# RainbowZL0/swin-unet-image-fusion

Measured on AMD Instinct MI355X. Metric: fused image-pairs/sec at 256x256, win=8, higher is better.
Workload: dtype bf16; 1 GPU; B=16/GPU 256x256 IR/visible pairs, win=8, 5-level Swin-UNet fusion forward (BASELINE configs[1]); global_batch=16, precision_mode=fast, residual_stream=fp32, hip_graph=True, steps_in_flight=3, kernel_schedule=throughput, collective=none, weights=random-init (numpy PCG64 recipe, seed 0)

## Files before the change

swin_unet_image_fusion_amd/csrc/kernels_attnproj.hip:

```cpp
#include "kernels_attnproj.h"

#include <cstdlib>

#include "win_frag.h"

namespace swf {
namespace {

using namespace wf;

constexpr int kC = 384, kD = 48, kHeads = 8, kNS = 3, kVRS = 72, kLDO = kC + 8;
constexpr size_t kVtBytes = size_t(kHeads) * kD * kVRS * 2, kBiasBytes = 2 * 2 * 16 * 64 * 4;
constexpr size_t kOBytes = size_t(2) * 64 * kLDO * 2;
constexpr size_t kXchBytes = size_t(8) * 16 * 64 * 4;
static_assert(kVtBytes + kBiasBytes <= kOBytes, "the O image covers the attention-phase images");
constexpr size_t kLds = kOBytes + kXchBytes;

struct ApDev {
    const f16* q[2]; const f16* k[2]; const f16* v[2];
    const bf16* wp_hi[2]; const bf16* wp_lo[2];
    const float* pbias[2]; const float* table[2];
    const float* res[2]; float* out[2];
    int B, H, W, shift;
};

#ifdef AP_PROBE
__device__ unsigned long long ap_probe[16];
#define AP_STAMP(i) do { if (blockIdx.x == AP_PROBE && blockIdx.y == 0 && blockIdx.z == 0 && threadIdx.x == 0) ap_probe[i] = wall_clock64(); } while (0)
#else
#define AP_STAMP(i) do { } while (0)
#endif

template <int WS>
__global__ __launch_bounds__(512) void attn_proj_kernel(ApDev a) {
    static_assert(WS == 7 || WS == 8, "window side");
    constexpr int C = kC, D = kD, VRS = kVRS, LDO = kLDO, TW = 2 * WS - 1;
    extern __shared__ __attribute__((aligned(16))) char smem[];
    f16* vt = reinterpret_cast<f16*>(smem);
    float* btile = reinterpret_cast<float*>(smem + kVtBytes);
    bf16* o_hi = reinterpret_cast<bf16*>(smem);
    bf16* o_lo = o_hi + 64 * LDO;

    const int tid = threadIdx.x, lane = tid & 63, wave = __builtin_amdgcn_readfirstlane(tid >> 6);
    const int r = lane & 31, hf = lane >> 5;
    const int H = a.H, W = a.W, nwx = W / WS, nwy = H / WS, npi = nwx * nwy;
    const int win = blockIdx.x, ns = blockIdx.y, st = blockIdx.z;
    const int b = win / npi, wrem = win - b * npi, wy = wrem / nwx, wx = wrem - wy * nwx;
    const int sh = a.shift ? WS / 2 : 0;
    auto padding = [](int t) { return WS != 8 && ((t >> 3) >= WS || (t & 7) >= WS); };
    auto tok_index = [&](int t) {
        const int ty = WS == 8 ? (t >> 3) : min(t >> 3, WS - 1), tx = WS == 8 ? (t & 7) : min(t & 7, WS - 1);
        int oy = wy * WS + ty + sh, ox = wx * WS + tx + sh;
        oy = oy >= H ? oy - H : oy;
        ox = ox >= W ? ox - W : ox;
        return (size_t)((b * H + oy) * W + ox);
    };

    AP_STAMP(0);
    const int head = wave;
    const f16* qg = a.q[st] + head * D + 8 * hf;
    const f16* kg = a.k[st] + head * D + 8 * hf;
    const size_t t0 = tok_index(r) * C, t1 = tok_index(32 + r) * C;
    u32x4 kf[2][3], qf[2][3], vrow[6];
#pragma unroll
    for (int ks = 0; ks < 3; ++ks) {
        kf[0][ks] = *reinterpret_cast<const u32x4*>(kg + t0 + 16 * ks);
        kf[1][ks] = *reinterpret_cast<const u32x4*>(kg + t1 + 16 * ks);
        qf[0][ks] = *reinterpret_cast<const u32x4*>(qg + t0 + 16 * ks);
        qf[1][ks] = *reinterpret_cast<const u32x4*>(qg + t1 + 16 * ks);
    }
    {
        const f16* vg = a.v[st] + tok_index(lane) * C + head * D;
#pragma unroll
        for (int j = 0; j < 6; ++j) vrow[j] = *reinterpret_cast<const u32x4*>(vg + 8 * j);
    }
    {
        const bool last_row = a.shift && wy == nwy - 1, last_col = a.shift && wx == nwx - 1;
        const float* tab = a.table[st];
#pragma unroll
// ... 43 lines not shown
#pragma unroll
        for (int i = 3; i < 16; i += 2) mx = max3f(mx, acc[0][i], acc[0][i + 1 < 16 ? i + 1 : i]);
#pragma unroll
        for (int i = 2; i < 16; i += 2) mx = max3f(mx, acc[1][i], acc[1][i + 1]);
        mx = max_halves(mx);
        float l = 0.f;
#pragma unroll
        for (int kt = 0; kt < 2; ++kt)
#pragma unroll
            for (int i = 0; i < 16; ++i) {
                acc[kt][i] = __builtin_amdgcn_exp2f(acc[kt][i] - mx);
                l += acc[kt][i];
            }
        l = sum_halves(l);
        o[qb][0] = zero16;
        o[qb][1] = zero16;
#pragma unroll
        for (int kt = 0; kt < 2; ++kt)
#pragma unroll
            for (int s2 = 0; s2 < 2; ++s2) {
                float p[8];
#pragma unroll
                for (int e = 0; e < 8; ++e) p[e] = acc[kt][8 * s2 + e];
                const u32x4 pf = pack8_f16(p);
                const u32x4 va0 = *reinterpret_cast<const u32x4*>(vth + r * VRS + kt * 32 + s2 * 16);
                const u32x4 va1 = *reinterpret_cast<const u32x4*>(vth + c1 * VRS + kt * 32 + s2 * 16);
                o[qb][0] = mfma_f16(va0, pf, o[qb][0]);
                o[qb][1] = mfma_f16(va1, pf, o[qb][1]);
            }
        inv[qb] = 1.0f / l;
    }

    AP_STAMP(4);
    const int ct = wave & 3, kh = wave >> 2, col0 = ns * (C / kNS) + 32 * ct;
    constexpr int KSH = C / 32;
    u32x4 wfh[KSH], wfl[KSH];
    {
        const size_t blk0 = (size_t)(col0 / 32) * (C / 16) + KSH * kh;
        const bf16* wh = a.wp_hi[st] + blk0 * 512 + lane * 8;
        const bf16* wl = a.wp_lo[st] + blk0 * 512 + lane * 8;
#pragma unroll
        for (int ks = 0; ks < KSH; ++ks) {
            wfh[ks] = *reinterpret_cast<const u32x4*>(wh + 512 * ks);
            wfl[ks] = *reinterpret_cast<const u32x4*>(wl + 512 * ks);
        }
    }
    const int t = 32 * kh + r;
    const size_t orow = tok_index(t) * C + col0 + 4 * hf;
    f32x4 rv[4], bv[4];
#pragma unroll
    for (int g = 0; g < 4; ++g) {
        rv[g] = *reinterpret_cast<const f32x4*>(a.res[st] + orow + 8 * g);
        bv[g] = a.pbias[st] ? *reinterpret_cast<const f32x4*>(a.pbias[st] + col0 + 8 * g + 4 * hf) : f32x4{0.f, 0.f, 0.f, 0.f};
    }
    __syncthreads();
#pragma unroll
    for (int qb = 0; qb < 2; ++qb)
#pragma unroll
        for (int mt = 0; mt < 2; ++mt)
#pragma unroll
            for (int g = 0; g < 4; ++g) {
                const int c = mt * 32 + 8 * g + 4 * hf;
                if (c < D) {
                    bf16x4 h4, l4;
#pragma unroll
                    for (int j = 0; j < 4; ++j) {
                        const float v = o[qb][mt][4 * g + j] * inv[qb];
                        h4[j] = (bf16)v;
                        l4[j] = (bf16)(v - (float)h4[j]);
                    }
                    *reinterpret_cast<bf16x4*>(o_hi + (32 * qb + r) * LDO + head * D + c) = h4;
                    *reinterpret_cast<bf16x4*>(o_lo + (32 * qb + r) * LDO + head * D + c) = l4;
                }
            }
    __syncthreads();
    AP_STAMP(5);

    f32x16 acc[2] = {zero16, zero16};
    {
        const bf16* oh = o_hi + r * LDO + (C / 2) * kh + 8 * hf;
        const bf16* ol = o_lo + r * LDO + (C / 2) * kh + 8 * hf;
#pragma unroll
        for (int ks = 0; ks < KSH; ++ks) {
            const u32x4 bh0 = *reinterpret_cast<const u32x4*>(oh + 16 * ks), bl0 = *reinterpret_cast<const u32x4*>(ol + 16 * ks);
            const u32x4 bh1 = *reinterpret_cast<const u32x4*>(oh + 32 * LDO + 16 * ks), bl1 = *reinterpret_cast<const u32x4*>(ol + 32 * LDO + 16 * ks);
            acc[0] = mma3(wfh[ks], wfl[ks], bh0, bl0, acc[0]);
            acc[1] = mma3(wfh[ks], wfl[ks], bh1, bl1, acc[1]);
        }
    }
    float* xch = reinterpret_cast<float*>(smem + kOBytes);
#pragma unroll
    for (int i = 0; i < 16; ++i) xch[(wave * 16 + i) * 64 + lane] = kh ? acc[0][i] : acc[1][i];
    __syncthreads();
    AP_STAMP(6);
    f32x16 mine = kh ? acc[1] : acc[0];
#pragma unroll
    for (int i = 0; i < 16; ++i) mine[i] += xch[((wave ^ 4) * 16 + i) * 64 + lane];
    if (padding(t)) return;
    float* out = a.out[st] + orow;
#pragma unroll
    for (int g = 0; g < 4; ++g) {
        f32x4 v = {mine[4 * g], mine[4 * g + 1], mine[4 * g + 2], mine[4 * g + 3]};
        v += bv[g];
        v += rv[g];
        *reinterpret_cast<f32x4*>(out + 8 * g) = v;
    }
    AP_STAMP(7);
}

}

bool attnproj_supported(const swf_block_desc& d) {
    static const bool off = debug_env("SWF_NO_ATTNPROJ") != nullptr;
    return !off && d.precision == SWF_PREC_FAST && d.attn.channels == kC && d.attn.heads == kHeads && d.attn.head_dim == kD &&
           d.attn.win_h == d.attn.win_w && (d.attn.win_h == 8 || d.attn.win_h == 7);
}

int launch_attnproj(const swf_block_desc& d, const AttnProjArgs& a, int nstream, hipStream_t stream) {
    const int ws = d.attn.win_h;
    if (!attnproj_supported(d) || a.H % ws || a.W % ws) return fail(SWF_ERR_UNSUPPORTED, "attnproj: shape not covered");
    if ((int64_t)a.B * a.H * a.W > INT32_MAX / kC) return fail(SWF_ERR_UNSUPPORTED, "attnproj: token count");
    ApDev dv{};
    for (int s = 0; s < nstream; ++s) {
        if (!a.q[s] || !a.k[s] || !a.v[s] || !a.wp_hi[s] || !a.wp_lo[s] || !a.table[s] || !a.res[s] || !a.out[s])
            return fail(SWF_ERR_NULL, "attnproj: NULL operand (stream %d)", s);
        dv.q[s] = reinterpret_cast<const f16*>(a.q[s]); dv.k[s] = reinterpret_cast<const f16*>(a.k[s]); dv.v[s] = reinterpret_cast<const f16*>(a.v[s]);
        dv.wp_hi[s] = reinterpret_cast<const bf16*>(a.wp_hi[s]); dv.wp_lo[s] = reinterpret_cast<const bf16*>(a.wp_lo[s]);
        dv.pbias[s] = a.pbias[s]; dv.table[s] = a.table[s]; dv.res[s] = a.res[s]; dv.out[s] = a.out[s];
    }
    dv.B = a.B; dv.H = a.H; dv.W = a.W; dv.shift = a.shift;
    const int nwin = a.B * (a.H / ws) * (a.W / ws);
    if (ws == 8) {
        SWF_TRY(raise_lds_limit<&attn_proj_kernel<8>>((int)kLds, "attn_proj"));
        hipLaunchKernelGGL((attn_proj_kernel<8>), dim3(nwin, kNS, nstream), dim3(512), kLds, stream, dv);
    } else {
        SWF_TRY(raise_lds_limit<&attn_proj_kernel<7>>((int)kLds, "attn_proj"));
        hipLaunchKernelGGL((attn_proj_kernel<7>), dim3(nwin, kNS, nstream), dim3(512), kLds, stream, dv);
    }
    return check_launch("attn_proj");
}

}
```

swin_unet_image_fusion_amd/csrc/kernels_deeppatch.h:

```cpp
#pragma once
#include "kernels_patch.h"

namespace swf {

bool deep_patch_supported(int decoder, int Cin, int Cout, int mh, int mw);
size_t deep_patch_packed_bytes(int decoder, int Cin, int Cout, int mh, int mw);
int pack_deep_patch(int decoder, int Cin, int Cout, int mh, int mw, const float* weight, void* dst, hipStream_t stream);
bool deep_patch_raw(int decoder, int Cin, int Cout, int mh, int mw);
struct DeepPatchExtra {
    const float* ln_gamma[2]; const float* ln_beta[2]; unsigned short* ln_hi[2]; unsigned short* ln_lo[2];
    const void* warm[2]; size_t warm_bytes;
};
int launch_deep_patch(const PatchFusedDesc& d, const void* const* packed, int nstream, hipStream_t stream, float* const* raw_out = nullptr,
                      const DeepPatchExtra* extra = nullptr);

int launch_deep_patch_finish(const PatchFusedDesc& d, float* const* raw, int nstream, hipStream_t stream, const DeepPatchExtra* extra = nullptr);

struct DeepQkvArgs {
    const unsigned short* xn_hi[2]; const unsigned short* xn_lo[2];
    const unsigned short* w_hi[2]; const unsigned short* w_lo[2];
    const float* bias[2][3];
    unsigned short* out[2][3];
    float qscale; int cross, M;
    int C;
};
bool deep_qkv_supported(const swf_block_desc& d);
int launch_deep_qkv(const DeepQkvArgs& q, int nstream, hipStream_t stream);

struct DeepProjArgs {
    const unsigned short* o_hi[2]; const unsigned short* o_lo[2];
    const unsigned short* w_hi[2]; const unsigned short* w_lo[2];
    const float* bias[2]; const float* res[2]; float* out[2];
    int M, C;
};
bool deep_proj_supported(const swf_block_desc& d);
int launch_deep_proj(const DeepProjArgs& q, int nstream, hipStream_t stream);

}
```

swin_unet_image_fusion_amd/csrc/kernels_deeppatch.hip:

```cpp
#include "kernels_deeppatch.h"

#include <cstdlib>

#include "kernels_qkvattn.h"
#include "win_frag.h"

namespace swf {
namespace {

using namespace wf;

struct DpArgs {
    const float* in[2]; float* out[2]; const float* skip[2];
    const bf16* w_hi[2]; const bf16* w_lo[2];
    const float* bias[2]; const float* gamma[2]; const float* beta[2];
    int B, H, W, Hm, Wm, Ho, Wo, M;
    const bf16* xh[2]; const bf16* xl[2]; const float* qb[2][3]; f16* qo[2][3]; float qscale; int cross;
    const float* ln_g[2]; const float* ln_b[2]; bf16* ln_hi[2]; bf16* ln_lo[2];
    const char* warm[2]; int warm_bytes;
};

#ifdef DP_PROBE
__device__ unsigned long long dp_probe[16];
#define DP_STAMP(i) do { if (blockIdx.x == DP_PROBE && blockIdx.y == 0 && threadIdx.x == 0) dp_probe[i] = wall_clock64(); } while (0)
// ... 516 lines not shown
    const int C = d.attn.channels;
    return !off && d.precision == SWF_PREC_FAST && d.attn.heads * d.attn.head_dim == C && (C == 384 || C == 192);
}

int launch_deep_proj(const DeepProjArgs& q, int nstream, hipStream_t stream) {
    if (q.M <= 0 || q.M > INT32_MAX / 2048) return fail(SWF_ERR_UNSUPPORTED, "deep_proj: token count");
    if (q.C != 192 && q.C != 384) return fail(SWF_ERR_UNSUPPORTED, "deep_proj: C=%d", q.C);
    DpArgs a{};
    for (int s = 0; s < nstream; ++s) {
        if (!q.o_hi[s] || !q.o_lo[s] || !q.w_hi[s] || !q.w_lo[s] || !q.out[s]) return fail(SWF_ERR_NULL, "deep_proj: NULL operand (stream %d)", s);
        a.xh[s] = reinterpret_cast<const bf16*>(q.o_hi[s]); a.xl[s] = reinterpret_cast<const bf16*>(q.o_lo[s]);
        a.w_hi[s] = reinterpret_cast<const bf16*>(q.w_hi[s]); a.w_lo[s] = reinterpret_cast<const bf16*>(q.w_lo[s]);
        a.bias[s] = q.bias[s]; a.skip[s] = q.res[s]; a.out[s] = q.out[s];
    }
    a.M = q.M;
    return q.C == 192 ? launch_t<192, 192, 2, 4, 3, 192>(a, nstream, stream) : launch_t<384, 192, 2, 4, 3, 384>(a, nstream, stream);
}

int launch_deep_qkv(const DeepQkvArgs& q, int nstream, hipStream_t stream) {
    if (q.M <= 0 || q.M > INT32_MAX / 2048) return fail(SWF_ERR_UNSUPPORTED, "deep_qkv: token count");
    DpArgs a{};
    for (int s = 0; s < nstream; ++s) {
        if (!q.xn_hi[s] || !q.xn_lo[s] || !q.w_hi[s] || !q.w_lo[s]) return fail(SWF_ERR_NULL, "deep_qkv: NULL operand (stream %d)", s);
        a.xh[s] = reinterpret_cast<const bf16*>(q.xn_hi[s]); a.xl[s] = reinterpret_cast<const bf16*>(q.xn_lo[s]);
        a.w_hi[s] = reinterpret_cast<const bf16*>(q.w_hi[s]); a.w_lo[s] = reinterpret_cast<const bf16*>(q.w_lo[s]);
        for (int i = 0; i < 3; ++i) {
            if (!q.out[s][i]) return fail(SWF_ERR_NULL, "deep_qkv: NULL output (stream %d)", s);
            a.qb[s][i] = q.bias[s][i]; a.qo[s][i] = reinterpret_cast<f16*>(q.out[s][i]);
        }
    }
    a.M = q.M; a.qscale = q.qscale; a.cross = q.cross && nstream == 2;
    if (q.C == 192) return launch_t<192, 192, 2, 4, 2, 576>(a, nstream, stream);
    if (q.C != 384) return fail(SWF_ERR_UNSUPPORTED, "deep_qkv: C=%d", q.C);
    return launch_t<384, 192, 2, 4, 2, 1152>(a, nstream, stream);
}

bool deep_patch_supported(int decoder, int Cin, int Cout, int mh, int mw) { return shape_index(decoder, Cin, Cout, mh, mw) >= 0; }
bool deep_patch_raw(int decoder, int Cin, int Cout, int mh, int mw) {
    const int i = shape_index(decoder, Cin, Cout, mh, mw);
    return i >= 0 && kShapes[i].raw;
}

size_t deep_patch_packed_bytes(int decoder, int Cin, int Cout, int mh, int mw) {
    const int i = shape_index(decoder, Cin, Cout, mh, mw);
    return i < 0 ? 0 : align_up((size_t)kShapes[i].K * kShapes[i].N * 4, 256);
}

int pack_deep_patch(int decoder, int Cin, int Cout, int mh, int mw, const float* weight, void* dst, hipStream_t stream) {
    const int i = shape_index(decoder, Cin, Cout, mh, mw);
    if (i < 0) return fail(SWF_ERR_UNSUPPORTED, "pack_deep_patch: shape not covered");
    const int K = kShapes[i].K, N = kShapes[i].N;
    bf16* hi = static_cast<bf16*>(dst);
    hipLaunchKernelGGL(dp_pack_kernel, dim3(256), dim3(256), 0, stream, weight, hi, hi + (size_t)N * K, N, K);
    return check_launch("pack_deep_patch");
}

int launch_deep_patch(const PatchFusedDesc& d, const void* const* packed, int nstream, hipStream_t stream, float* const* raw_out,
                      const DeepPatchExtra* extra) {
    const int i = shape_index(d.decoder, d.Cin, d.Cout, d.mh, d.mw);
    if (i < 0) return fail(SWF_ERR_UNSUPPORTED, "deep_patch: shape not covered");
    if (d.M <= 0 || d.M > INT32_MAX / 1024 || (int64_t)d.B * d.H * d.W * d.Cin > INT32_MAX) return fail(SWF_ERR_UNSUPPORTED, "deep_patch: map too large");
    const int K = kShapes[i].K, N = kShapes[i].N;
    DpArgs a{};
    for (int s = 0; s < nstream; ++s) {
        if (!packed || !packed[s] || !d.in[s] || !d.out[s] || !d.gamma[s] || !d.beta[s]) return fail(SWF_ERR_NULL, "deep_patch: NULL operand (stream %d)", s);
        if (kShapes[i].raw && (!raw_out || !raw_out[s])) return fail(SWF_ERR_NULL, "deep_patch: this shape needs the conv output buffer (stream %d)", s);
// ... 25 lines not shown
```

swin_unet_image_fusion_amd/csrc/kernels_patchrr.hip:

```cpp
#include "kernels_patchrr.h"

#include <algorithm>

#include "win_frag.h"

namespace swf {
namespace {

using namespace wf;

struct PrrArgs {
    const float* in[2]; float* out[2]; const float* skip[2]; const char* packed[2];
    int B, H, W, Cin;
    int mh, mw, Hm, Wm;
    int Ho, Wo;
    int K, N, Cout, M;
};

template <int KS, int NT>
struct PRR {
    static constexpr int NFRAG = NT * KS * 2;
    static constexpr int NV = NT * 16;
    static constexpr size_t p_vec = size_t(NFRAG) * 1024;
    static constexpr size_t p_total = p_vec + size_t(3) * 2 * NV * 4;
};

template <int KS, int NT, int DEC, int CIN1, int TPW>
__global__ __launch_bounds__(256) void patch_rr_kernel(PrrArgs a) {
    using P = PRR<KS, NT>;
    constexpr int NV = P::NV;
    __shared__ float lvec[3 * 2 * NV];
    const int s = blockIdx.y, tid = threadIdx.x, lane = tid & 63, wave = tid >> 6;
    const int r = lane & 31, hf = lane >> 5;
    fill_vectors<3 * NV / 4, 256>(lvec, a.packed[s] + P::p_vec, a.packed[s] + P::p_vec + (3 * NV / 4) * 16, tid);
    const __amdgpu_buffer_rsrc_t wrs = __builtin_amdgcn_make_buffer_rsrc(const_cast<char*>(a.packed[s]), 0, (int)P::p_total, 0x00020000);
    const unsigned loff = (unsigned)lane * 16u;
    auto WA = [&](int nt, int ks, int hl) {
        return __builtin_bit_cast(u32x4, __builtin_amdgcn_raw_buffer_load_b128(wrs, loff, ((nt * KS + ks) * 2 + hl) * 1024, 0));
    };
    __syncthreads();
    const float* vbias = lvec + hf * NV;
    const float* vgam = lvec + 2 * NV + hf * NV;
    const float* vbet = lvec + 4 * NV + hf * NV;
    const float* in = a.in[s];
    const int K = a.K, N = a.N, Cin = a.Cin;
    const float invN = 1.0f / (float)N;
    const f32x16 zero16 = {0.f, 0.f, 0.f, 0.f, 0.f, 0.f, 0.f, 0.f, 0.f, 0.f, 0.f, 0.f, 0.f, 0.f, 0.f, 0.f};

    const int ngroup = (a.M + 32 * TPW - 1) / (32 * TPW);
    for (int grp = blockIdx.x * 4 + wave; grp < ngroup; grp += gridDim.x * 4) {
        int tok[TPW], base[TPW][4];
        bool live[TPW];
#pragma unroll
        for (int u = 0; u < TPW; ++u) {
            const int t = (grp * TPW + u) * 32 + r;
            live[u] = t < a.M;
            const int tc = live[u] ? t : a.M - 1;
            tok[u] = tc;
            if constexpr (DEC) {
                const int mx = tc % a.Wm, t2 = tc / a.Wm, my = t2 % a.Hm, b = t2 / a.Hm;
                base[u][0] = ((b * a.H + my) * a.W + mx) * Cin;
                base[u][1] = base[u][2] = base[u][3] = 0;
            } else {
// ... 54 lines not shown
        auto dec_offsets = [&](int u) {
            const int t = tok[u];
            const int mx = t % a.Wm, t2 = t / a.Wm, my = t2 % a.Hm, b = t2 / a.Hm;
            int pq = 0, c = 4 * hf;
            while (c >= a.Cout) { c -= a.Cout; ++pq; }
#pragma unroll
            for (int nt = 0; nt < NT; ++nt)
#pragma unroll
                for (int g = 0; g < 4; ++g) {
                    const int yy = my * 2 + (pq >> 1), xx = mx * 2 + (pq & 1);
                    const bool ok = live[u] && 32 * nt + 8 * g + 4 * hf < N && yy < a.Ho && xx < a.Wo;
                    oidx[u][nt][g] = ok ? ((b * a.Ho + yy) * a.Wo + xx) * a.Cout + c : -1;
                    c += 8;
                    while (c >= a.Cout) { c -= a.Cout; ++pq; }
                }
        };
        auto load_skips = [&](int u) {
#pragma unroll
            for (int nt = 0; nt < NT; ++nt)
#pragma unroll
                for (int g = 0; g < 4; ++g)
                    skv[u][nt][g] = (a.skip[s] && oidx[u][nt][g] >= 0) ? *reinterpret_cast<const float4*>(a.skip[s] + oidx[u][nt][g])
                                                                       : make_float4(0.f, 0.f, 0.f, 0.f);
        };
        if constexpr (DEC_VEC) {
            if (a.Cout > 1) {
#pragma unroll
                for (int u = 0; u < TPW; ++u) {
                    dec_offsets(u);
                    if constexpr (SKIP_EARLY) load_skips(u);
                }
            }
        }
        u32x4 wr[2][NT][2];
        SWF_WF_FENCE();
#pragma unroll
        for (int nt = 0; nt < NT; ++nt) { wr[0][nt][0] = WA(nt, 0, 0); wr[0][nt][1] = WA(nt, 0, 1); }
#pragma unroll
        for (int ks = 0; ks < KS; ++ks) {
            if (ks + 1 < KS) {
#pragma unroll
                for (int nt = 0; nt < NT; ++nt) { wr[(ks + 1) & 1][nt][0] = WA(nt, ks + 1, 0); wr[(ks + 1) & 1][nt][1] = WA(nt, ks + 1, 1); }
            }
            SWF_WF_FENCE();
            u32x4 bh[TPW], bl[TPW];
#pragma unroll
            for (int u = 0; u < TPW; ++u) split8(xin[u][ks], bh[u], bl[u]);
#pragma unroll
            for (int nt = 0; nt < NT; ++nt)
#pragma unroll
                for (int u = 0; u < TPW; ++u) acc[u][nt] = mma3(wr[ks & 1][nt][0], wr[ks & 1][nt][1], bh[u], bl[u], acc[u][nt]);
        }
#pragma unroll
        for (int u = 0; u < TPW; ++u) {
            float sum = 0.f;
#pragma unroll
            for (int nt = 0; nt < NT; ++nt)
#pragma unroll
                for (int i = 0; i < 16; ++i) {
                    acc[u][nt][i] += vbias[nt * 16 + i];
                    sum += acc[u][nt][i];
                }
            const float mean = sum_halves(sum) * invN;
            float q = 0.f;
#pragma unroll
            for (int nt = 0; nt < NT; ++nt)
#pragma unroll
                for (int i = 0; i < 16; ++i) {
                    const float d = acc[u][nt][i] - mean;
                    q += (32 * nt + rho(i, hf) < N) ? d * d : 0.f;
                }
            const float rstd = __builtin_amdgcn_rsqf(sum_halves(q) * invN + 1e-5f);
            const int t = tok[u];
            if constexpr (DEC_VEC) {
                if (a.Cout > 1) {
                    if constexpr (!SKIP_EARLY) load_skips(u);
                }
            }
#pragma unroll
            for (int nt = 0; nt < NT; ++nt)
#pragma unroll
                for (int g = 0; g < 4; ++g) {
                    const int n0 = 32 * nt + 8 * g + 4 * hf;
                    if (n0 < N) {
// ... 39 lines not shown
    const int gtid = blockIdx.x * blockDim.x + threadIdx.x, gsz = gridDim.x * blockDim.x;
    for (int idx = gtid; idx < P::NFRAG * 512; idx += gsz) {
        const int f = idx >> 9, lane = (idx >> 3) & 63, e = idx & 7, r = lane & 31, hf = lane >> 5;
        const int hl = f & 1, ks = (f >> 1) % KS, nt = f / (2 * KS);
        const int n = 32 * nt + r, k = 16 * ks + 8 * hf + e;
        const float val = (n < a.N && k < a.K) ? a.w[(int64_t)n * a.K + k] : 0.f;
        const bf16 hi = (bf16)val;
        reinterpret_cast<bf16*>(a.dst)[idx] = hl ? (bf16)(val - (float)hi) : hi;
    }
    float* vec = reinterpret_cast<float*>(a.dst + P::p_vec);
    for (int i = gtid; i < 3 * 2 * P::NV; i += gsz) {
        const int which = i / (2 * P::NV), hf = (i / P::NV) & 1, j = i % P::NV, nt = j >> 4, reg = j & 15;
        const int n = 32 * nt + rho(reg, hf);
        const float* src = which == 0 ? a.bias : which == 1 ? a.gamma : a.beta;
        vec[i] = (n < a.N && src) ? src[n] : 0.f;
    }
}

bool shape_class(int decoder, int Cin, int Cout, int mh, int mw, int* ks, int* nt) {
    if (mh != 2 || mw != 2 || Cin <= 0 || Cout <= 0) return false;
    const int K = decoder ? Cin : 4 * Cin, N = decoder ? 4 * Cout : Cout;
    if (decoder) {
        if (Cin % 8 || !(Cout == 1 || Cout % 4 == 0)) return false;
    } else {
        if (!(Cin == 1 || Cin % 8 == 0) || Cout % 4) return false;
    }
    *ks = (K + 15) / 16;
    *nt = (N + 31) / 32;
    const int k = *ks, n = *nt;
    if (decoder) return (k == 2 && n == 1) || (k == 3 && n == 3) || (k == 6 && n == 6);
    return (k == 1 && n == 1 && Cin == 1) || (k == 6 && n == 2) || (k == 12 && n == 3);
}

template <int KS, int NT, int DEC, int CIN1, int TPW>
int launch_t(const PrrArgs& a, int nstream, hipStream_t stream) {
    const int ngroup = (a.M + 32 * TPW - 1) / (32 * TPW);
    const int gx = std::max(1, std::min((ngroup + 3) / 4, 8 * num_cus() / nstream));
    hipLaunchKernelGGL((patch_rr_kernel<KS, NT, DEC, CIN1, TPW>), dim3(gx, nstream), dim3(256), 0, stream, a);
    return check_launch("patch_rr");
}

}

bool patch_rr_supported(int decoder, int Cin, int Cout, int mh, int mw) {
    int ks, nt;
    return shape_class(decoder, Cin, Cout, mh, mw, &ks, &nt);
}

size_t patch_rr_packed_bytes(int decoder, int Cin, int Cout, int mh, int mw) {
    int ks, nt;
    if (!shape_class(decoder, Cin, Cout, mh, mw, &ks, &nt)) return 0;
    return align_up(size_t(nt) * ks * 2 * 1024 + size_t(3) * 2 * nt * 16 * 4, 256);
}

int pack_patch_rr(int decoder, int Cin, int Cout, int mh, int mw, const float* weight, const float* bias, const float* gamma,
                  const float* beta, void* dst, hipStream_t stream) {
    int ks, nt;
    if (!shape_class(decoder, Cin, Cout, mh, mw, &ks, &nt)) return fail(SWF_ERR_UNSUPPORTED, "pack_patch_rr: shape not covered");
    PrrPackArgs a{weight, bias, gamma, beta, static_cast<char*>(dst), decoder ? Cin : 4 * Cin, decoder ? 4 * Cout : Cout};
#define SWF_PRR_PACK(KS_, NT_) if (ks == KS_ && nt == NT_) { hipLaunchKernelGGL((patch_rr_pack_kernel<KS_, NT_>), dim3(32), dim3(256), 0, stream, a); return check_launch("pack_patch_rr"); }
    SWF_PRR_PACK(1, 1) SWF_PRR_PACK(2, 1) SWF_PRR_PACK(3, 3) SWF_PRR_PACK(6, 2) SWF_PRR_PACK(6, 6) SWF_PRR_PACK(12, 3)
#undef SWF_PRR_PACK
    return fail(SWF_ERR_UNSUPPORTED, "pack_patch_rr: shape class");
}

int launch_patch_rr(const PatchFusedDesc& d, const void* const* packed, int nstream, hipStream_t stream) {
    int ks, nt;
    if (!shape_class(d.decoder, d.Cin, d.Cout, d.mh, d.mw, &ks, &nt)) return fail(SWF_ERR_UNSUPPORTED, "patch_rr: shape not covered");
    if (d.M <= 0 || d.M > INT32_MAX - 64) return fail(SWF_ERR_UNSUPPORTED, "patch_rr: token count");
    const int64_t in_elems = (int64_t)d.B * d.H * d.W * d.Cin;
    const int64_t out_elems = d.decoder ? (int64_t)d.B * d.Ho * d.Wo * d.Cout : d.M * (int64_t)d.N;
    if (in_elems >= (int64_t(1) << 31) || out_elems >= (int64_t(1) << 31)) return fail(SWF_ERR_UNSUPPORTED, "patch_rr: tensor too large");
    PrrArgs a{};
    uintptr_t bits = 0;
    for (int s = 0; s < nstream; ++s) {
        if (!packed || !packed[s]) return fail(SWF_ERR_NULL, "patch_rr: packed image missing");
        a.in[s] = d.in[s]; a.out[s] = d.out[s]; a.skip[s] = d.skip[s]; a.packed[s] = static_cast<const char*>(packed[s]);
        bits |= reinterpret_cast<uintptr_t>(d.in[s]) | reinterpret_cast<uintptr_t>(d.out[s]) | reinterpret_cast<uintptr_t>(d.skip[s]) |
                reinterpret_cast<uintptr_t>(packed[s]);
    }
    if (bits % 16) return fail(SWF_ERR_UNSUPPORTED, "patch_rr: tensors must be 16-byte aligned");
    a.B = d.B; a.H = d.H; a.W = d.W; a.Cin = d.Cin; a.mh = d.mh; a.mw = d.mw; a.Hm = d.Hm; a.Wm = d.Wm; a.Ho = d.Ho; a.Wo = d.Wo;
    a.K = d.K; a.N = d.N; a.Cout = d.Cout; a.M = (int)d.M;
    if (!d.decoder) {
        if (ks == 1 && nt == 1 && d.Cin == 1) return launch_t<1, 1, 0, 1, 2>(a, nstream, stream);
        if (ks == 6 && nt == 2) return launch_t<6, 2, 0, 0, 2>(a, nstream, stream);
        if (ks == 12 && nt == 3) return launch_t<12, 3, 0, 0, 1>(a, nstream, stream);
    } else {
        if (ks == 2 && nt == 1) return launch_t<2, 1, 1, 0, 2>(a, nstream, stream);
        if (ks == 3 && nt == 3) return launch_t<3, 3, 1, 0, 1>(a, nstream, stream);
        if (ks == 6 && nt == 6) return launch_t<6, 6, 1, 0, 1>(a, nstream, stream);
    }
    return fail(SWF_ERR_UNSUPPORTED, "patch_rr: no instantiation for k-steps %d, tiles %d (decoder %d)", ks, nt, d.decoder);
}

}
```

swin_unet_image_fusion_amd/csrc/swf_api.hip:

```cpp
#include <algorithm>
#include <cmath>
#include <mutex>
#include <string>
#include <vector>

#include "kernels_generic.h"
#include <cstdlib>
#include "kernels_window.h"
#include "kernels_bwd.h"
#include "kernels_dropout.h"
#include "kernels_loss.h"
#include "kernels_fidelity.h"
#include "kernels_metrics.h"
#include "kernels_optim.h"
#include "kernels_deep.h"
#include "kernels_patch.h"
#include "kernels_patchrr.h"
#include "kernels_deeppatch.h"
#include "kernels_mlp.h"
#include "kernels_qkvattn.h"
#include "kernels_attnproj.h"

namespace swf {

// ... 282 lines not shown
    }
    const bool fused_attn = fused_attn_shape && wv[0].qa && (nstream == 1 || wv[1].qa);
    const bool fold_proj = proj_fused && fused_attn && pp[0]->attn.proj.bias && (nstream == 1 || pp[1]->attn.proj.bias);
    if (fused_attn) {
        QkvAttnArgs qa{};
        for (int s = 0; s < nstream; ++s) {
            qa.packed[s] = wv[s].qa; qa.xn_hi[s] = b.xn_hi[s]; qa.xn_lo[s] = b.xn_lo[s]; qa.o_hi[s] = b.o_hi[s]; qa.o_lo[s] = b.o_lo[s];
            if (fold_proj) { qa.part[0][s] = b.part[0][s]; qa.part[1][s] = b.part[1][s]; }
        }
        qa.B = B; qa.H = H; qa.W = W; qa.shift = desc->attn.shift; qa.cross = cross;
        SWF_TRY(launch_qkvattn(*desc, qa, nstream, stream));
        trace_block(route, SWF_BLOCK_DEEP_QKVATTN | (fold_proj ? SWF_BLOCK_DEEP_FOLD_PROJ : 0));
    }
    SpGemmBatch gq{};
    for (int s = 0; s < nstream; ++s) {
        const int kvs = cross ? 1 - s : s;
        const swf_linear* lin[3] = {&pp[s]->attn.q, &pp[s]->attn.k, &pp[s]->attn.v};
        const bf16_raw* wh[3] = {wv[s].q_hi, wv[s].k_hi, wv[s].v_hi};
        const bf16_raw* wl[3] = {wv[s].q_lo, wv[s].k_lo, wv[s].v_lo};
        for (int i = 0; i < 3; ++i) {
            const int src = i == 0 ? s : kvs;
            gq.p[s * 3 + i] = SpGemmProb{b.xn_hi[src], b.xn_lo[src], wh[i], wl[i], lin[i]->bias, nullptr, nullptr, b.qkv[s][i], nullptr};
        }
    }
    gq.qscale = 1.4426950408889634f / std::sqrt((float)desc->attn.head_dim);
    const bool deep_qkv = !fused_attn && HD == C && deep_qkv_supported(*desc) && wv[0].qkvf_hi && (nstream == 1 || wv[1].qkvf_hi);
    if (deep_qkv) {
        DeepQkvArgs dq{};
        for (int s = 0; s < nstream; ++s) {
            dq.xn_hi[s] = b.xn_hi[s]; dq.xn_lo[s] = b.xn_lo[s]; dq.w_hi[s] = wv[s].qkvf_hi; dq.w_lo[s] = wv[s].qkvf_lo;
            dq.bias[s][0] = pp[s]->attn.q.bias; dq.bias[s][1] = pp[s]->attn.k.bias; dq.bias[s][2] = pp[s]->attn.v.bias;
            for (int i = 0; i < 3; ++i) dq.out[s][i] = b.qkv[s][i];
        }
        dq.qscale = gq.qscale; dq.cross = cross; dq.M = (int)N; dq.C = C;
        SWF_TRY(launch_deep_qkv(dq, nstream, stream));
        trace_block(route, SWF_BLOCK_DEEP_QKV);
    }
    if (!fused_attn && !deep_qkv) SWF_TRY(launch_gemm_sp(gq, 3 * nstream, (int)N, HD, C, HD, SP_EPI_QKV16, stream));
    const bool attn_proj = !fused_attn && HD == C && attnproj_supported(*desc) && wv[0].pf_hi && (nstream == 1 || wv[1].pf_hi);
    if (attn_proj) {
        AttnProjArgs ap{};
        for (int s = 0; s < nstream; ++s) {
            ap.q[s] = b.qkv[s][0]; ap.k[s] = b.qkv[s][1]; ap.v[s] = b.qkv[s][2];
            ap.wp_hi[s] = wv[s].pf_hi; ap.wp_lo[s] = wv[s].pf_lo; ap.pbias[s] = pp[s]->attn.proj.bias; ap.table[s] = pp[s]->attn.bias_table;
            ap.res[s] = xin[s]; ap.out[s] = xout[s];
        }
        ap.B = B; ap.H = H; ap.W = W; ap.shift = desc->attn.shift;
        SWF_TRY(launch_attnproj(*desc, ap, nstream, stream));
        trace_block(route, SWF_BLOCK_DEEP_ATTNPROJ);
    }
    if (!fused_attn && !attn_proj) {
        const bf16_raw* qq[2] = {b.qkv[0][0], b.qkv[1][0]};
        const bf16_raw* kk[2] = {b.qkv[0][1], b.qkv[1][1]};
        const bf16_raw* vv[2] = {b.qkv[0][2], b.qkv[1][2]};
        const float* tt[2] = {pp[0]->attn.bias_table, nstream == 2 ? pp[1]->attn.bias_table : nullptr};
        if (desc->attn.win_h == 16) {
            SWF_TRY(launch_attn_core_mfma16(nullptr, nullptr, nullptr, nullptr, tt, nstream, HD, HD, HD, HD, B, H, W, desc->attn.heads,
                                            desc->attn.head_dim, desc->attn.shift, nullptr, stream, b.o_hi, b.o_lo, qq, kk, vv));
            trace_block(route, SWF_BLOCK_DEEP_CORE16);
        } else
            SWF_TRY(launch_attn_core_mfma(nullptr, nullptr, nullptr, nullptr, tt, nstream, HD, HD, HD, HD, B, H, W, desc->attn.heads,
                                          desc->attn.head_dim, desc->attn.shift, stream, b.o_hi, b.o_lo, qq, kk, vv, desc->attn.win_h));
    }
    SpGemmBatch gp{};
    gp.scratch = b.sk; gp.scratch_floats = b.sk_floats;
    for (int s = 0; s < nstream; ++s)
        gp.p[s] = SpGemmProb{b.o_hi[s], b.o_lo[s], wv[s].p_hi, wv[s].p_lo, pp[s]->attn.proj.bias, xin[s], xout[s], nullptr, nullptr};
// ... 1932 lines not shown
```

Baseline: 8914 pairs/s.

## Loop all projection thirds per workgroup, widen deep QKV tile, deepen patch weight ring

Under the throughput schedule, the attention+projection kernel now computes all three output-column thirds in one workgroup. This avoids recomputing attention three times across grid.y, and it prefetches the next third's weight fragments while the current third's MFMAs run. The deep QKV launch picks a wider 384-column tile under the throughput schedule. The patch_rr kernel gains a configurable weight-fragment ring depth with deeper prefetch and scheduling barriers. The trade-off is fewer workgroups and more register pressure in exchange for much less redundant attention work.

```diff
diff --git a/swin_unet_image_fusion_amd/csrc/kernels_attnproj.hip b/swin_unet_image_fusion_amd/csrc/kernels_attnproj.hip
--- a/swin_unet_image_fusion_amd/csrc/kernels_attnproj.hip
+++ b/swin_unet_image_fusion_amd/csrc/kernels_attnproj.hip
@@ -31,9 +31,10 @@
 #define AP_STAMP(i) do { } while (0)
 #endif
 
-template <int WS>
+template <int WS, int NSW>
 __global__ __launch_bounds__(512) void attn_proj_kernel(ApDev a) {
     static_assert(WS == 7 || WS == 8, "window side");
+    static_assert(NSW == 1 || NSW == kNS, "thirds per workgroup");
     constexpr int C = kC, D = kD, VRS = kVRS, LDO = kLDO, TW = 2 * WS - 1;
     extern __shared__ __attribute__((aligned(16))) char smem[];
     f16* vt = reinterpret_cast<f16*>(smem);
@@ -44,7 +45,7 @@
     const int tid = threadIdx.x, lane = tid & 63, wave = __builtin_amdgcn_readfirstlane(tid >> 6);
     const int r = lane & 31, hf = lane >> 5;
     const int H = a.H, W = a.W, nwx = W / WS, nwy = H / WS, npi = nwx * nwy;
-    const int win = blockIdx.x, ns = blockIdx.y, st = blockIdx.z;
+    const int win = blockIdx.x, ns0 = NSW == 1 ? (int)blockIdx.y : 0, st = blockIdx.z;
     const int b = win / npi, wrem = win - b * npi, wy = wrem / nwx, wx = wrem - wy * nwx;
     const int sh = a.shift ? WS / 2 : 0;
     auto padding = [](int t) { return WS != 8 && ((t >> 3) >= WS || (t & 7) >= WS); };
@@ -154,27 +155,28 @@
     }
 
     AP_STAMP(4);
-    const int ct = wave & 3, kh = wave >> 2, col0 = ns * (C / kNS) + 32 * ct;
+    const int ct = wave & 3, kh = wave >> 2;
     constexpr int KSH = C / 32;
     u32x4 wfh[KSH], wfl[KSH];
-    {
-        const size_t blk0 = (size_t)(col0 / 32) * (C / 16) + KSH * kh;
-        const bf16* wh = a.wp_hi[st] + blk0 * 512 + lane * 8;
-        const bf16* wl = a.wp_lo[st] + blk0 * 512 + lane * 8;
-#pragma unroll
-        for (int ks = 0; ks < KSH; ++ks) {
-            wfh[ks] = *reinterpret_cast<const u32x4*>(wh + 512 * ks);
-            wfl[ks] = *reinterpret_cast<const u32x4*>(wl + 512 * ks);
-        }
-    }
+    auto wp_frag = [&](int third, int ks) {
+        const size_t blk = (size_t)(third * (C / kNS) / 32 + ct) * (C / 16) + KSH * kh + ks;
+        wfh[ks] = *reinterpret_cast<const u32x4*>(a.wp_hi[st] + blk * 512 + lane * 8);
+        wfl[ks] = *reinterpret_cast<const u32x4*>(a.wp_lo[st] + blk * 512 + lane * 8);
+    };
+#pragma unroll
+    for (int ks = 0; ks < KSH; ++ks) wp_frag(ns0, ks);
     const int t = 32 * kh + r;
-    const size_t orow = tok_index(t) * C + col0 + 4 * hf;
+    const size_t trow = tok_index(t) * C + 4 * hf;
     f32x4 rv[4], bv[4];
-#pragma unroll
-    for (int g = 0; g < 4; ++g) {
-        rv[g] = *reinterpret_cast<const f32x4*>(a.res[st] + orow + 8 * g);
-        bv[g] = a.pbias[st] ? *reinterpret_cast<const f32x4*>(a.pbias[st] + col0 + 8 * g + 4 * hf) : f32x4{0.f, 0.f, 0.f, 0.f};
-    }
+    auto row_operands = [&](int third) {
+        const int col0 = third * (C / kNS) + 32 * ct;
+#pragma unroll
+        for (int g = 0; g < 4; ++g) {
+            rv[g] = *reinterpret_cast<const f32x4*>(a.res[st] + trow + col0 + 8 * g);
+            bv[g] = a.pbias[st] ? *reinterpret_cast<const f32x4*>(a.pbias[st] + col0 + 8 * g + 4 * hf) : f32x4{0.f, 0.f, 0.f, 0.f};
+        }
+    };
+    row_operands(ns0);
     __syncthreads();
 #pragma unroll
     for (int qb = 0; qb < 2; ++qb)
@@ -198,36 +200,67 @@
     __syncthreads();
     AP_STAMP(5);
 
-    f32x16 acc[2] = {zero16, zero16};
-    {
-        const bf16* oh = o_hi + r * LDO + (C / 2) * kh + 8 * hf;
-        const bf16* ol = o_lo + r * LDO + (C / 2) * kh + 8 * hf;
-#pragma unroll
-        for (int ks = 0; ks < KSH; ++ks) {
-            const u32x4 bh0 = *reinterpret_cast<const u32x4*>(oh + 16 * ks), bl0 = *reinterpret_cast<const u32x4*>(ol + 16 * ks);
-            const u32x4 bh1 = *reinterpret_cast<const u32x4*>(oh + 32 * LDO + 16 * ks), bl1 = *reinterpret_cast<const u32x4*>(ol + 32 * LDO + 16 * ks);
-            acc[0] = mma3(wfh[ks], wfl[ks], bh0, bl0, acc[0]);
-            acc[1] = mma3(wfh[ks], wfl[ks], bh1, bl1, acc[1]);
-        }
-    }
     float* xch = reinterpret_cast<float*>(smem + kOBytes);
-#pragma unroll
-    for (int i = 0; i < 16; ++i) xch[(wave * 16 + i) * 64 + lane] = kh ? acc[0][i] : acc[1][i];
-    __syncthreads();
-    AP_STAMP(6);
-    f32x16 mine = kh ? acc[1] : acc[0];
-#pragma unroll
-    for (int i = 0; i < 16; ++i) mine[i] += xch[((wave ^ 4) * 16 + i) * 64 + lane];
-    if (padding(t)) return;
-    float* out = a.out[st] + orow;
-#pragma unroll
-    for (int g = 0; g < 4; ++g) {
-        f32x4 v = {mine[4 * g], mine[4 * g + 1], mine[4 * g + 2], mine[4 * g + 3]};
-        v += bv[g];
-        v += rv[g];
-        *reinterpret_cast<f32x4*>(out + 8 * g) = v;
-    }
-    AP_STAMP(7);
+    const bf16* oh = o_hi + r * LDO + (C / 2) * kh + 8 * hf;
+    const bf16* ol = o_lo + r * LDO + (C / 2) * kh + 8 * hf;
+#pragma unroll
+    for (int i3 = 0; i3 < NSW; ++i3) {
+        const int ns = ns0 + i3;
+        if (i3 > 0) {
+            __syncthreads();
+            row_operands(ns);
+        }
+        f32x16 acc[2] = {zero16, zero16};
+        if constexpr (NSW > 1) {
+            u32x4 nb[4] = {*reinterpret_cast<const u32x4*>(oh), *reinterpret_cast<const u32x4*>(ol),
+                           *reinterpret_cast<const u32x4*>(oh + 32 * LDO), *reinterpret_cast<const u32x4*>(ol + 32 * LDO)};
+#pragma unroll
+            for (int ks = 0; ks < KSH; ++ks) {
+                const u32x4 bh0 = nb[0], bl0 = nb[1], bh1 = nb[2], bl1 = nb[3];
+                if (ks + 1 < KSH) {
+                    nb[0] = *reinterpret_cast<const u32x4*>(oh + 16 * (ks + 1)); nb[1] = *reinterpret_cast<const u32x4*>(ol + 16 * (ks + 1));
+                    nb[2] = *reinterpret_cast<const u32x4*>(oh + 32 * LDO + 16 * (ks + 1)); nb[3] = *reinterpret_cast<const u32x4*>(ol + 32 * LDO + 16 * (ks + 1));
+                }
+                acc[0] = mma3(wfh[ks], wfl[ks], bh0, bl0, acc[0]);
+                acc[1] = mma3(wfh[ks], wfl[ks], bh1, bl1, acc[1]);
+                if (i3 + 1 < NSW) wp_frag(ns + 1, ks);
+                __builtin_amdgcn_sched_barrier(0);
+            }
+        } else {
+#pragma unroll
+            for (int ks = 0; ks < KSH; ++ks) {
+                const u32x4 bh0 = *reinterpret_cast<const u32x4*>(oh + 16 * ks), bl0 = *reinterpret_cast<const u32x4*>(ol + 16 * ks);
+                const u32x4 bh1 = *reinterpret_cast<const u32x4*>(oh + 32 * LDO + 16 * ks), bl1 = *reinterpret_cast<const u32x4*>(ol + 32 * LDO + 16 * ks);
+                acc[0] = mma3(wfh[ks], wfl[ks], bh0, bl0, acc[0]);
+                acc[1] = mma3(wfh[ks], wfl[ks], bh1, bl1, acc[1]);
+            }
+        }
+#pragma unroll
+        for (int i = 0; i < 16; ++i) xch[(wave * 16 + i) * 64 + lane] = kh ? acc[0][i] : acc[1][i];
+        __syncthreads();
+        AP_STAMP(6 + 2 * i3);
+        f32x16 mine = kh ? acc[1] : acc[0];
+#pragma unroll
+        for (int i = 0; i < 16; ++i) mine[i] += xch[((wave ^ 4) * 16 + i) * 64 + lane];
+        if (!padding(t)) {
+            float* out = a.out[st] + trow + ns * (C / kNS) + 32 * ct;
+#pragma unroll
+            for (int g = 0; g < 4; ++g) {
+                f32x4 v = {mine[4 * g], mine[4 * g + 1], mine[4 * g + 2], mine[4 * g + 3]};
+                v += bv[g];
+                v += rv[g];
+                *reinterpret_cast<f32x4*>(out + 8 * g) = v;
+            }
+        }
+        AP_STAMP(7 + 2 * i3);
+    }
+}
+
+template <int WS, int NSW>
+int launch_t(const ApDev& dv, int nwin, int nstream, hipStream_t stream) {
+    SWF_TRY((raise_lds_limit<&attn_proj_kernel<WS, NSW>>((int)kLds, "attn_proj")));
+    hipLaunchKernelGGL((attn_proj_kernel<WS, NSW>), dim3(nwin, kNS / NSW, nstream), dim3(512), kLds, stream, dv);
+    return check_launch("attn_proj");
 }
 
 }
@@ -252,14 +285,9 @@
     }
     dv.B = a.B; dv.H = a.H; dv.W = a.W; dv.shift = a.shift;
     const int nwin = a.B * (a.H / ws) * (a.W / ws);
-    if (ws == 8) {
-        SWF_TRY(raise_lds_limit<&attn_proj_kernel<8>>((int)kLds, "attn_proj"));
-        hipLaunchKernelGGL((attn_proj_kernel<8>), dim3(nwin, kNS, nstream), dim3(512), kLds, stream, dv);
-    } else {
-        SWF_TRY(raise_lds_limit<&attn_proj_kernel<7>>((int)kLds, "attn_proj"));
-        hipLaunchKernelGGL((attn_proj_kernel<7>), dim3(nwin, kNS, nstream), dim3(512), kLds, stream, dv);
-    }
-    return check_launch("attn_proj");
-}
-
-}
+    const bool all_thirds = d.schedule == SWF_SCHED_THROUGHPUT;
+    if (ws == 8) return all_thirds ? launch_t<8, kNS>(dv, nwin, nstream, stream) : launch_t<8, 1>(dv, nwin, nstream, stream);
+    return all_thirds ? launch_t<7, kNS>(dv, nwin, nstream, stream) : launch_t<7, 1>(dv, nwin, nstream, stream);
+}
+
+}
diff --git a/swin_unet_image_fusion_amd/csrc/kernels_deeppatch.h b/swin_unet_image_fusion_amd/csrc/kernels_deeppatch.h
--- a/swin_unet_image_fusion_amd/csrc/kernels_deeppatch.h
+++ b/swin_unet_image_fusion_amd/csrc/kernels_deeppatch.h
@@ -23,6 +23,7 @@
     unsigned short* out[2][3];
     float qscale; int cross, M;
     int C;
+    int schedule;
 };
 bool deep_qkv_supported(const swf_block_desc& d);
 int launch_deep_qkv(const DeepQkvArgs& q, int nstream, hipStream_t stream);
diff --git a/swin_unet_image_fusion_amd/csrc/kernels_deeppatch.hip b/swin_unet_image_fusion_amd/csrc/kernels_deeppatch.hip
--- a/swin_unet_image_fusion_amd/csrc/kernels_deeppatch.hip
+++ b/swin_unet_image_fusion_amd/csrc/kernels_deeppatch.hip
@@ -572,6 +572,7 @@
     a.M = q.M; a.qscale = q.qscale; a.cross = q.cross && nstream == 2;
     if (q.C == 192) return launch_t<192, 192, 2, 4, 2, 576>(a, nstream, stream);
     if (q.C != 384) return fail(SWF_ERR_UNSUPPORTED, "deep_qkv: C=%d", q.C);
+    if (q.schedule == SWF_SCHED_THROUGHPUT) return launch_t<384, 384, 2, 8, 2, 1152>(a, nstream, stream);
     return launch_t<384, 192, 2, 4, 2, 1152>(a, nstream, stream);
 }
 
diff --git a/swin_unet_image_fusion_amd/csrc/kernels_patchrr.hip b/swin_unet_image_fusion_amd/csrc/kernels_patchrr.hip
--- a/swin_unet_image_fusion_amd/csrc/kernels_patchrr.hip
+++ b/swin_unet_image_fusion_amd/csrc/kernels_patchrr.hip
@@ -25,10 +25,13 @@
     static constexpr size_t p_total = p_vec + size_t(3) * 2 * NV * 4;
 };
 
-template <int KS, int NT, int DEC, int CIN1, int TPW>
+template <int KS, int NT, int DEC, int CIN1, int TPW, int RD>
 __global__ __launch_bounds__(256) void patch_rr_kernel(PrrArgs a) {
     using P = PRR<KS, NT>;
     constexpr int NV = P::NV;
+    static_assert(RD >= 1 && RD <= KS && (RD >= 2 || KS == 1), "ring depth");
+    constexpr int PRE = RD == KS ? KS : RD - 1;
+    constexpr bool PIN = PRE > 1;
     __shared__ float lvec[3 * 2 * NV];
     const int s = blockIdx.y, tid = threadIdx.x, lane = tid & 63, wave = tid >> 6;
     const int r = lane & 31, hf = lane >> 5;
@@ -149,24 +152,28 @@
                 }
             }
         }
-        u32x4 wr[2][NT][2];
+        u32x4 wr[RD][NT][2];
         SWF_WF_FENCE();
 #pragma unroll
-        for (int nt = 0; nt < NT; ++nt) { wr[0][nt][0] = WA(nt, 0, 0); wr[0][nt][1] = WA(nt, 0, 1); }
+        for (int ks = 0; ks < PRE; ++ks)
+#pragma unroll
+            for (int nt = 0; nt < NT; ++nt) { wr[ks % RD][nt][0] = WA(nt, ks, 0); wr[ks % RD][nt][1] = WA(nt, ks, 1); }
+        if constexpr (PIN) __builtin_amdgcn_sched_barrier(0);
 #pragma unroll
         for (int ks = 0; ks < KS; ++ks) {
-            if (ks + 1 < KS) {
-#pragma unroll
-                for (int nt = 0; nt < NT; ++nt) { wr[(ks + 1) & 1][nt][0] = WA(nt, ks + 1, 0); wr[(ks + 1) & 1][nt][1] = WA(nt, ks + 1, 1); }
+            if (ks + PRE < KS) {
+#pragma unroll
+                for (int nt = 0; nt < NT; ++nt) { wr[(ks + PRE) % RD][nt][0] = WA(nt, ks + PRE, 0); wr[(ks + PRE) % RD][nt][1] = WA(nt, ks + PRE, 1); }
             }
             SWF_WF_FENCE();
+            if constexpr (PIN) __builtin_amdgcn_sched_barrier(0);
             u32x4 bh[TPW], bl[TPW];
 #pragma unroll
             for (int u = 0; u < TPW; ++u) split8(xin[u][ks], bh[u], bl[u]);
 #pragma unroll
             for (int nt = 0; nt < NT; ++nt)
 #pragma unroll
-                for (int u = 0; u < TPW; ++u) acc[u][nt] = mma3(wr[ks & 1][nt][0], wr[ks & 1][nt][1], bh[u], bl[u], acc[u][nt]);
+                for (int u = 0; u < TPW; ++u) acc[u][nt] = mma3(wr[ks % RD][nt][0], wr[ks % RD][nt][1], bh[u], bl[u], acc[u][nt]);
         }
 #pragma unroll
         for (int u = 0; u < TPW; ++u) {
@@ -272,11 +279,11 @@
     return (k == 1 && n == 1 && Cin == 1) || (k == 6 && n == 2) || (k == 12 && n == 3);
 }
 
-template <int KS, int NT, int DEC, int CIN1, int TPW>
+template <int KS, int NT, int DEC, int CIN1, int TPW, int RD>
 int launch_t(const PrrArgs& a, int nstream, hipStream_t stream) {
     const int ngroup = (a.M + 32 * TPW - 1) / (32 * TPW);
     const int gx = std::max(1, std::min((ngroup + 3) / 4, 8 * num_cus() / nstream));
-    hipLaunchKernelGGL((patch_rr_kernel<KS, NT, DEC, CIN1, TPW>), dim3(gx, nstream), dim3(256), 0, stream, a);
+    hipLaunchKernelGGL((patch_rr_kernel<KS, NT, DEC, CIN1, TPW, RD>), dim3(gx, nstream), dim3(256), 0, stream, a);
     return check_launch("patch_rr");
 }
 
@@ -323,13 +330,13 @@
     a.B = d.B; a.H = d.H; a.W = d.W; a.Cin = d.Cin; a.mh = d.mh; a.mw = d.mw; a.Hm = d.Hm; a.Wm = d.Wm; a.Ho = d.Ho; a.Wo = d.Wo;
     a.K = d.K; a.N = d.N; a.Cout = d.Cout; a.M = (int)d.M;
     if (!d.decoder) {
-        if (ks == 1 && nt == 1 && d.Cin == 1) return launch_t<1, 1, 0, 1, 2>(a, nstream, stream);
-        if (ks == 6 && nt == 2) return launch_t<6, 2, 0, 0, 2>(a, nstream, stream);
-        if (ks == 12 && nt == 3) return launch_t<12, 3, 0, 0, 1>(a, nstream, stream);
+        if (ks == 1 && nt == 1 && d.Cin == 1) return launch_t<1, 1, 0, 1, 2, 1>(a, nstream, stream);
+        if (ks == 6 && nt == 2) return launch_t<6, 2, 0, 0, 2, 3>(a, nstream, stream);
+        if (ks == 12 && nt == 3) return launch_t<12, 3, 0, 0, 1, 3>(a, nstream, stream);
     } else {
-        if (ks == 2 && nt == 1) return launch_t<2, 1, 1, 0, 2>(a, nstream, stream);
-        if (ks == 3 && nt == 3) return launch_t<3, 3, 1, 0, 1>(a, nstream, stream);
-        if (ks == 6 && nt == 6) return launch_t<6, 6, 1, 0, 1>(a, nstream, stream);
+        if (ks == 2 && nt == 1) return launch_t<2, 1, 1, 0, 2, 2>(a, nstream, stream);
+        if (ks == 3 && nt == 3) return launch_t<3, 3, 1, 0, 1, 2>(a, nstream, stream);
+        if (ks == 6 && nt == 6) return launch_t<6, 6, 1, 0, 1, 3>(a, nstream, stream);
     }
     return fail(SWF_ERR_UNSUPPORTED, "patch_rr: no instantiation for k-steps %d, tiles %d (decoder %d)", ks, nt, d.decoder);
 }
diff --git a/swin_unet_image_fusion_amd/csrc/swf_api.hip b/swin_unet_image_fusion_amd/csrc/swf_api.hip
--- a/swin_unet_image_fusion_amd/csrc/swf_api.hip
+++ b/swin_unet_image_fusion_amd/csrc/swf_api.hip
@@ -338,7 +338,7 @@
             dq.bias[s][0] = pp[s]->attn.q.bias; dq.bias[s][1] = pp[s]->attn.k.bias; dq.bias[s][2] = pp[s]->attn.v.bias;
             for (int i = 0; i < 3; ++i) dq.out[s][i] = b.qkv[s][i];
         }
-        dq.qscale = gq.qscale; dq.cross = cross; dq.M = (int)N; dq.C = C;
+        dq.qscale = gq.qscale; dq.cross = cross; dq.M = (int)N; dq.C = C; dq.schedule = desc->schedule;
         SWF_TRY(launch_deep_qkv(dq, nstream, stream));
         trace_block(route, SWF_BLOCK_DEEP_QKV);
     }
```

Measured after the change: 9173 pairs/s (median of 6 runs). 1.03x the previous value.
